# rkin100g/Nerf-Replication

Measured on AMD Instinct MI355X. Metric: rays/sec (800x800, 64+128 samples), higher is better.
Workload: dtype f32; 1 GPU; lego-shaped 800x800 frame = 640000 pinhole rays, 64 coarse + 128 fine hierarchical samples, 8+1-layer W=256 NeRF x2, seeded synthetic weights (latest.pth unavailable offline); BASELINE.json configs[1]; parallelism=ray-tile shard x1 (each rank generates and renders only its tile) + 1 all_gather

## Files before the change

nerf_replication_amd/csrc/nerf_frame.hip.inc:

```
#include "nerf_host.h"

namespace {

__global__ void nerf_occupancy_tally_kernel(const int* __restrict__ count, long long all, long long* __restrict__ evaluated) {
  *evaluated += count ? (long long)*count : all;
}

}

extern "C" {

static constexpr int64_t kRenderBlockRays = 1 << 20;
static int64_t render_block_rays() {
  const char* env = getenv("NERF_RENDER_BLOCK_RAYS");
  constexpr long long kMax = 0x7fffffff / (NERF_N_SAMPLES + NERF_N_IMPORTANCE);
  if (env) { const long long v = atoll(env); if (v >= 64) return (int64_t)(v < kMax ? v : kMax); }
  return kRenderBlockRays;
}

struct RenderWorkspace {
  float* raw_c; float* t_sorted = nullptr; float* raw_f = nullptr; uint8_t* valid = nullptr; int* index; int* count; float* t_jit = nullptr;
  uint8_t* valid_c = nullptr; int* index_c = nullptr;
  int64_t bytes;
  RenderWorkspace(void* base, int64_t n_rays, int32_t n_importance, int32_t fast_sampling, bool stochastic, bool occupancy = false) {
    Carver c(base);
    const int64_t S = NERF_N_SAMPLES + NERF_N_IMPORTANCE;
    raw_c = c.take<float>(n_rays * NERF_N_SAMPLES * 4);
    if (n_importance) {
      t_sorted = c.take<float>(n_rays * S);
      raw_f = c.take<float>(n_rays * S * 4);
    }
    if (n_importance && (fast_sampling || occupancy)) {
      valid = c.take<uint8_t>(n_rays * S);
      index = c.take<int>(n_rays * S);
    } else {
      index = c.take<int>(n_rays);
    }
    count = c.take<int>(1);
    if (stochastic) t_jit = c.take<float>(n_rays * NERF_N_SAMPLES);
    if (occupancy) {
      valid_c = c.take<uint8_t>(n_rays * NERF_N_SAMPLES);
      index_c = c.take<int>(n_rays * NERF_N_SAMPLES);
    }
    bytes = c.bytes();
  }
};
static int64_t render_workspace_bytes(int64_t n_rays_frame, int32_t n_importance, int32_t fast_sampling, bool stochastic,
                                      bool occupancy = false) {
  if (n_rays_frame < 0) return -1;
  const int64_t n_rays = n_rays_frame < render_block_rays() ? n_rays_frame : render_block_rays();
  return RenderWorkspace(nullptr, n_rays, n_importance, fast_sampling, stochastic, occupancy).bytes;
}

struct RenderOccupancy {
  const uint32_t* coarse; const uint32_t* fine;
  int32_t dims[3]; float box_min[3], inv_step[3];
  long long* evaluated;
};
static int occupancy_tally(const int* count, long long all, long long* evaluated, hipStream_t st) {
  return NERF_LAUNCH(nerf_occupancy_tally_kernel, dim3(1), dim3(1), st, count, all, evaluated);
}
int64_t nerf_render_workspace_bytes(int64_t n_rays_frame, int32_t n_importance, int32_t fast_sampling) {
  return render_workspace_bytes(n_rays_frame, n_importance, fast_sampling, false);
}
int64_t nerf_render_stochastic_workspace_bytes(int64_t n_rays_frame, int32_t n_importance) {
  return render_workspace_bytes(n_rays_frame, n_importance, 0, true);
}

static int32_t render_frame(const char* entry, const float* rays_o, const float* rays_d, int64_t n_rays, const void* packed_coarse,
                            const void* packed_fine, const float* t_coarse, const float* u, const float* jitter, const float* u_rays,
                            bool stochastic, int32_t n_importance, int32_t white_bkgd, int32_t precision, int32_t fast_sampling,
                            float weights_threshold, void* workspace, int64_t workspace_bytes, float* rgb, float* depth, void* stream,
                            const RenderOccupancy* occ = nullptr) {
  if (n_rays < 0) return fail(NERF_ERR_INVALID_ARG, "%s: bad size", entry);
  if (n_importance != 0 && n_importance != NERF_N_IMPORTANCE)
    return fail(NERF_ERR_INVALID_ARG, "%s: n_importance must be 0 or 128", entry);
  if (n_rays == 0) return NERF_OK;
  if (!rays_o || !rays_d || !packed_coarse || !t_coarse || !rgb || !depth || !workspace ||
      (n_importance && (!packed_fine || !u)))
    return fail(NERF_ERR_INVALID_ARG, "%s: null argument", entry);
  if (workspace_bytes < render_workspace_bytes(n_rays, n_importance, fast_sampling, stochastic, occ != nullptr))
    return fail(NERF_ERR_WORKSPACE, "%s: workspace too small", entry);
  const int64_t S = NERF_N_SAMPLES + NERF_N_IMPORTANCE;
  if (fast_sampling && n_importance && n_rays > (int64_t)0x7fffffff / S)
    return fail(NERF_ERR_INVALID_ARG, "%s: fast_sampling handles at most 11 184 810 rays per call "
                                      "(n_rays * 192 point ids must fit in int32): split the frame", entry);
  hipStream_t st = (hipStream_t)stream;
  const int64_t B = render_block_rays();
  for (int64_t r0 = 0; r0 < n_rays; r0 += B) {
    const int64_t nb = n_rays - r0 < B ? n_rays - r0 : B;
    const float* o = rays_o + 3 * r0;
    const float* d = rays_d + 3 * r0;
    float* rgb_b = rgb + 3 * r0;
    float* depth_b = depth + r0;
    const RenderWorkspace w(workspace, nb, n_importance, fast_sampling, stochastic, occ != nullptr);
    auto list_pass = [&](const uint8_t* valid, long long np, int* index, float* raw) -> int {
      if (hipMemsetAsync(w.count, 0, sizeof(int), st) != hipSuccess ||
          hipMemsetAsync(raw, 0, (size_t)(np * 4 * (int64_t)sizeof(float)), st) != hipSuccess)
        return fail(NERF_ERR_HIP, "%s: memset failed", entry);
      return NERF_LAUNCH(nerf_compact_kernel, dim3((unsigned)((np + 255) / 256)), dim3(256), st, valid, np, index, w.count);
    };
    auto tally = [&](int pass, bool listed, long long all) -> int {
      return occ && occ->evaluated ? occupancy_tally(listed ? w.count : nullptr, all, occ->evaluated + pass, st) : NERF_OK;
    };
    const float* tc = t_coarse;
    int64_t tcs = 0;
    int rc;
    if (jitter) {
      rc = nerf_stratified_samples(t_coarse, jitter + NERF_N_SAMPLES * r0, nb, w.t_jit, stream);
      if (rc) return rc;
      tc = w.t_jit; tcs = NERF_N_SAMPLES;
    }
    const bool cull_c = occ && occ->coarse;
    if (cull_c) {
      rc = nerf_occupancy_mark(o, d, tc, tcs, nb, NERF_N_SAMPLES, occ->coarse, occ->dims, occ->box_min, occ->inv_step, 0, w.valid_c, stream);
      if (rc) return rc;
      rc = list_pass(w.valid_c, nb * NERF_N_SAMPLES, w.index_c, w.raw_c);
      if (rc) return rc;
    }
    const bool fp16 = precision == NERF_PREC_F16 || precision == NERF_PREC_F16S;
    const bool exact_coarse = fp16 && fast_sampling && n_importance;
    rc = forward_rays(entry, o, d, tc, tcs, nb, NERF_N_SAMPLES, exact_coarse ? (const char*)packed_coarse + nerf::kF16PackedBytes : packed_coarse,
                      w.raw_c, false, nullptr, n_importance != 0, false, exact_coarse ? NERF_PREC_F32X : precision, stream,
                      cull_c ? w.index_c : nullptr, cull_c ? w.count : nullptr);
    if (rc) return rc;
    rc = tally(0, cull_c, nb * NERF_N_SAMPLES);
    if (rc) return rc;
    const bool guard = fp16 && nb <= (int64_t)0x7fffffff / S;
    auto far_plane_guard = [&](const float* tvals, int64_t stride, int32_t S_, const void* packed_f16, float* raw) -> int {
      if (const int r2 = NERF_LAUNCH(nerf_last_sample_index_kernel, dim3((unsigned)((nb + 255) / 256)), dim3(256), st, w.index, w.count,
                                     (long long)nb, S_)) return r2;
      return forward_rays(entry, o, d, tvals, stride, nb, S_, (const char*)packed_f16 + nerf::kF16PackedBytes, raw, false, nullptr, false,
                          false, NERF_PREC_F32X, stream, w.index, w.count);
    };
    if (n_importance == 0) {
      if (guard) {
        rc = far_plane_guard(tc, tcs, NERF_N_SAMPLES, packed_coarse, w.raw_c);
        if (rc) return rc;
      }
      rc = nerf_composite(w.raw_c, tc, tcs, nb, NERF_N_SAMPLES, white_bkgd, rgb_b, depth_b, nullptr, stream);
      if (rc) return rc;
      continue;
    }
    rc = nerf_sample_fine_rays(w.raw_c, tc, tcs, u_rays ? u_rays + NERF_N_IMPORTANCE * r0 : u, u_rays ? NERF_N_IMPORTANCE : 0, nb, w.t_sorted,
                               nullptr, fast_sampling ? w.valid : nullptr, fast_sampling ? weights_threshold : 0.f, fast_sampling ? 0.45f : 0.f,
                               stream);
    if (rc) return rc;
    const bool cull_f = occ && occ->fine;
    if (cull_f) {
      rc = nerf_occupancy_mark(o, d, w.t_sorted, S, nb, (int32_t)S, occ->fine, occ->dims, occ->box_min, occ->inv_step, fast_sampling != 0, w.valid,
                               stream);
      if (rc) return rc;
    }
    if (!fast_sampling && !cull_f) {
      rc = forward_rays(entry, o, d, w.t_sorted, S, nb, (int32_t)S, packed_fine, w.raw_f, false, nullptr, false, true, precision, stream);
      if (rc) return rc;
      if (guard) {
        rc = far_plane_guard(w.t_sorted, S, (int32_t)S, packed_fine, w.raw_f);
        if (rc) return rc;
      }
    } else {
      rc = list_pass(w.valid, nb * S, w.index, w.raw_f);
      if (rc) return rc;
      rc = forward_rays(entry, o, d, w.t_sorted, S, nb, (int32_t)S, packed_fine, w.raw_f, false, nullptr, false, true, precision, stream,
                        w.index, w.count);
      if (rc) return rc;
    }
    rc = tally(1, fast_sampling || cull_f, nb * S);
    if (rc) return rc;
    if (guard && fast_sampling && !cull_f) {
      rc = far_plane_guard(w.t_sorted, S, (int32_t)S, packed_fine, w.raw_f);
      if (rc) return rc;
    }
    rc = nerf_composite(w.raw_f, w.t_sorted, S, nb, (int32_t)S, white_bkgd, rgb_b, depth_b, nullptr, stream);
    if (rc) return rc;
  }
  return NERF_OK;
}

int32_t nerf_render_forward(const float* rays_o, const float* rays_d, int64_t n_rays,
                            const void* packed_coarse, const void* packed_fine,
                            const float* t_coarse, const float* u, int32_t n_importance,
                            int32_t white_bkgd, int32_t precision, int32_t fast_sampling,
                            float weights_threshold, void* workspace,
                            int64_t workspace_bytes, float* rgb, float* depth, void* stream) {
  return render_frame("nerf_render_forward", rays_o, rays_d, n_rays, packed_coarse, packed_fine, t_coarse, u, nullptr, nullptr, false,
                      n_importance, white_bkgd, precision, fast_sampling, weights_threshold, workspace, workspace_bytes, rgb, depth, stream);
}

int32_t nerf_render_forward_stochastic(const float* rays_o, const float* rays_d, int64_t n_rays,
                                       const void* packed_coarse, const void* packed_fine,
                                       const float* t_coarse, const float* u, const float* jitter, const float* u_rays,
                                       int32_t n_importance, int32_t white_bkgd, int32_t precision, int32_t fast_sampling,
                                       float weights_threshold, void* workspace, int64_t workspace_bytes,
                                       float* rgb, float* depth, void* stream) {
  if (precision != NERF_PREC_F32 && precision != NERF_PREC_F32X)
    return fail(NERF_ERR_INVALID_ARG, "%s", "nerf_render_forward_stochastic: precision must be f32 or f32x");
  if (fast_sampling) return fail(NERF_ERR_INVALID_ARG, "%s", "nerf_render_forward_stochastic: fast_sampling is not supported");
  return render_frame("nerf_render_forward_stochastic", rays_o, rays_d, n_rays, packed_coarse, packed_fine, t_coarse, u, jitter, u_rays,
                      true, n_importance, white_bkgd, precision, 0, weights_threshold, workspace, workspace_bytes, rgb, depth, stream);
}

}
```

nerf_replication_amd/csrc/nerf_mlp_common.h:

```cpp
#pragma once
#include <hip/hip_runtime.h>
#include <utility>

#include "nerf_layout.h"

typedef float f32x16 __attribute__((ext_vector_type(16)));
typedef float f32x4 __attribute__((ext_vector_type(4)));
typedef float f32x2 __attribute__((ext_vector_type(2)));
typedef unsigned u32x4 __attribute__((ext_vector_type(4)));
typedef _Float16 h8 __attribute__((ext_vector_type(8)));
typedef _Float16 h4 __attribute__((ext_vector_type(4)));
typedef _Float16 h2 __attribute__((ext_vector_type(2)));

typedef __attribute__((address_space(3))) void lds_void;
typedef const __attribute__((address_space(1))) void gbl_void;
typedef __attribute__((address_space(3))) char lds_char;
typedef __attribute__((address_space(3))) f32x4 lds_f32x4;
typedef const __attribute__((address_space(3))) float lds_cfloat;
typedef const __attribute__((address_space(3))) f32x2 lds_cf32x2;
typedef const __attribute__((address_space(3))) f32x4 lds_cf32x4;
typedef const __attribute__((address_space(3))) h8 lds_ch8;

constexpr int kF16Waves = 8;
constexpr int kF16Threads = kF16Waves * 64;
constexpr int kF16TilePts = kF16Waves * 32;
constexpr int kF16RingSlots = 4;
constexpr int kF16LdsBytes = nerf::kF16ConstBytes + kF16RingSlots * nerf::kF16ChunkBytes;
constexpr int kXWaves = 4;
constexpr int kXThreads = kXWaves * 64;
constexpr int kXTilePts = kXWaves * 32;

__device__ __forceinline__ f32x16 mfma32(float a, float b, f32x16 c) {
  return __builtin_amdgcn_mfma_f32_32x32x2f32(a, b, c, 0, 0, 0);
}
__device__ __forceinline__ f32x16 mfma16(h8 a, h8 b, f32x16 c) {
  return __builtin_amdgcn_mfma_f32_32x32x16_f16(a, b, c, 0, 0, 0);
}

__device__ __forceinline__ void sincos_cw(float x, float& s, float& c) {
  const float n = rintf(x * 0.636619772367581343f);
  float r = fmaf(n, -1.5703125f, x);
  r = fmaf(n, -4.837512969970703125e-4f, r);
  r = fmaf(n, -7.54978995489188216e-8f, r);
  const float r2 = r * r;
  const float sp = fmaf(r * r2, fmaf(r2, fmaf(r2, -1.9515295891e-4f, 8.3321608736e-3f), -1.6666654611e-1f), r);
  const float cp = fmaf(r2 * r2, fmaf(r2, fmaf(r2, 2.443315711809948e-5f, -1.388731625493765e-3f), 4.166664568298827e-2f),
                        fmaf(r2, -0.5f, 1.0f));
  const int q = (int)n;
  const float ss = (q & 1) ? cp : sp;
  const float cc = (q & 1) ? sp : cp;
  s = (q & 2) ? -ss : ss;
  c = ((q + 1) & 2) ? -cc : cc;
}

__device__ __forceinline__ int uniform_load_i32(const int* p) {
  return *(const __attribute__((address_space(4))) int*)p;
}

template <class F, int... I>
__device__ __forceinline__ void static_for_impl(F&& f, std::integer_sequence<int, I...>) { (f(std::integral_constant<int, I>{}), ...); }
template <int N, class F>
__device__ __forceinline__ void static_for(F&& f) { static_for_impl(f, std::make_integer_sequence<int, N>{}); }

struct MlpArgs {
  const float* pts;
  const float* rays_o;
  const float* rays_d;
  const float* viewdirs;
  const float* tvals;
  long long t_ray_stride;
  long long n_points;
  int n_samples;
  const float* packed;
  float* raw;
  const int* index;
  const int* count;
  float* save;
  int skip_dead_colour;
  int density_only;
  const float* fold;
  int skip_dead_ksteps;
  int skip_dead_groups;
};

struct TrainSave {
  static constexpr int kPe = 64, kDpe = 32;
  static constexpr long long pad32(long long P) { return (P + 31) & ~31LL; }
  static constexpr long long off_pe(long long P) { return 0; }
  static constexpr long long off_dpe(long long P) { return pad32(P) * 64; }
  static constexpr long long off_h(long long P, int l) { return pad32(P) * (96 + 256LL * l); }
  static constexpr long long off_f(long long P) { return pad32(P) * (96 + 2048); }
  static constexpr long long off_hv(long long P) { return pad32(P) * (96 + 2304); }
  static constexpr int kMasked = 9;
  static constexpr long long off_bits(long long P) { return pad32(P) * (96 + 2304 + 128); }
  static constexpr long long bits_block(long long tile, int which) { return ((tile * kMasked + which) * 64) * 4; }
  static constexpr long long off_stamp(long long P) { return off_bits(P) + (pad32(P) / 32) * kMasked * 256; }
  static constexpr long long floats(long long P) { return off_stamp(P) + 4; }
};

struct BwdArgs {
  const float* rays_o; const float* rays_d; const float* tvals; long long t_ray_stride;
  long long n_points; int n_samples;
  const float* packed_bwd;
  const float* draw;
  const float* save;
  float* gsave;
  float* g_t;
  const float* pts;
  float* g_x;
  int density_only;
  const int* live_tiles;
  const int* n_live;
};

struct TrainGrad {
  static constexpr long long off_gzv(long long P) { return 0; }
  static constexpr long long off_gf(long long P) { return TrainSave::pad32(P) * 128; }
  static constexpr long long off_gz(long long P, int l) { return TrainSave::pad32(P) * (384 + 256LL * (7 - l)); }
  static constexpr long long n_tiles(long long P) { return TrainSave::pad32(P) / 32; }
  static constexpr long long off_flags(long long P) { return TrainSave::pad32(P) * (384 + 2048); }
  static constexpr long long off_live(long long P) { return off_flags(P) + ((n_tiles(P) + 3) & ~3LL); }
  static constexpr long long off_count(long long P) { return off_live(P) + ((n_tiles(P) + 3) & ~3LL); }
  static constexpr long long floats(long long P) { return off_count(P) + 4; }
};
```

nerf_replication_amd/csrc/nerf_mlp_f32.hip.inc:

```

#include "nerf_mlp_common.h"

#ifndef NERF_F32_WG_WAVES
#define NERF_F32_WG_WAVES 1
#endif
#ifndef NERF_F32_HACK_NOBIAS
#define NERF_F32_HACK_NOBIAS 0
#endif
#ifndef NERF_F32_HACK_NOSAVE
#define NERF_F32_HACK_NOSAVE 0
#endif
#ifndef NERF_BWD_HACK_NOMASK
#define NERF_BWD_HACK_NOMASK 0
#endif

constexpr int kTailFloats = 3072;
static_assert(nerf::kOffHeadBias - nerf::kOffBias == kTailFloats, "LDS tail = biases + views bias + head weights");
template <int NT>
__device__ __forceinline__ void load_bias(f32x16 (&acc)[NT], lds_cfloat* bias_h) {
  lds_cf32x4* b = reinterpret_cast<lds_cf32x4*>(bias_h);
#pragma unroll
  for (int j = 0; j < NT; ++j) {
#pragma unroll
    for (int q = 0; q < 4; ++q) {
      f32x4 v = NERF_F32_HACK_NOBIAS ? f32x4{0.f, 0.f, 0.f, 0.f} : b[j * 4 + q];
      acc[j][4 * q + 0] = v.x; acc[j][4 * q + 1] = v.y; acc[j][4 * q + 2] = v.z; acc[j][4 * q + 3] = v.w;
    }
  }
}

constexpr int kRing = 16;
constexpr int kPF = 8;

#ifndef NERF_SAVE_TAPS
#define NERF_SAVE_TAPS 1
#endif
struct NoTap { static constexpr bool kIsTap = false; __device__ __forceinline__ void operator()(int, int, const f32x16&) const {} };
struct SignBits { unsigned w0 = 0u, w1 = 0u, w2 = 0u, w3 = 0u; };
template <bool GRAD, bool BITS = false>
struct StoreTap {
  static constexpr bool kIsTap = true;
  float* row;
  SignBits* sb;
  __device__ __forceinline__ void operator()(int t, int q, const f32x16& Xt) const {
    f32x4 v;
    v.x = Xt[4 * q + 0]; v.y = Xt[4 * q + 1]; v.z = Xt[4 * q + 2]; v.w = Xt[4 * q + 3];
    asm volatile("" : "+v"(v));
    if (!(GRAD ? 0 : NERF_F32_HACK_NOSAVE)) {
      *reinterpret_cast<f32x4*>(row + 32 * t + 8 * q) = v;
    }
    if constexpr (BITS) {
      auto nz = [](float x) { const unsigned u = __float_as_uint(x); return u < 1u ? u : 1u; };
      const unsigned m = (nz(v.x) | (nz(v.y) << 1) | (nz(v.z) << 2) | (nz(v.w) << 3)) << (16 * (t & 1) + 4 * q);
      switch (t >> 1) {
        case 0: sb->w0 |= m; break;
        case 1: sb->w1 |= m; break;
        case 2: sb->w2 |= m; break;
        default: sb->w3 |= m; break;
      }
    }
  }
};
template <bool ON, bool BITS>
__device__ __forceinline__ auto save_tap(float* row, SignBits* sb) {
  if constexpr (ON && NERF_SAVE_TAPS) return StoreTap<false, BITS>{row, sb};
  else return NoTap{};
}

struct AStream {
  const char* base;
  unsigned voff;
  f32x4 ring[kRing];
};
template <int N, int K = 0>
__device__ __forceinline__ void astream_load(AStream& as, int first, int slot0) {
  if constexpr (K < N) {
    const char* b = as.base + (long long)(first + (K & ~3)) * 1024;
    asm volatile("global_load_dwordx4 %0, %1, %2 offset:%3"
                 : "=&v"(as.ring[(slot0 + K) % kRing]) : "v"(as.voff), "s"(b), "n"((K & 3) * 1024) : "memory");
    astream_load<N, K + 1>(as, first, slot0);
  }
}
template <int K>
__device__ __forceinline__ void astream_load_one(AStream& as, int first, int slot0) {
  const char* b = as.base + (long long)(first + (K & ~3)) * 1024;
  asm volatile("global_load_dwordx4 %0, %1, %2 offset:%3"
               : "=&v"(as.ring[(slot0 + K) % kRing]) : "v"(as.voff), "s"(b), "n"((K & 3) * 1024) : "memory");
}
__device__ __forceinline__ void astream_fetch_from(AStream& as, unsigned& P) {
  const char* b0 = as.base + (long long)P * (8 * 1024);
  const char* b1 = b0 + 4096;
  asm volatile("s_cmp_eq_u32 %[P], 0\n\t"
               "s_cbranch_scc1 .Lpre_done_%=\n\t"
               "s_waitcnt vmcnt(0)\n\t"
               "s_bitcmp1_b32 %[P], 0\n\t"
               "s_cbranch_scc1 .Lpre_odd_%=\n\t"
               "global_load_dwordx4 %0, %[vo], %[b0]\n\t"
               "global_load_dwordx4 %1, %[vo], %[b0] offset:1024\n\t"
               "global_load_dwordx4 %2, %[vo], %[b0] offset:2048\n\t"
               "global_load_dwordx4 %3, %[vo], %[b0] offset:3072\n\t"
               "global_load_dwordx4 %4, %[vo], %[b1]\n\t"
               "global_load_dwordx4 %5, %[vo], %[b1] offset:1024\n\t"
               "global_load_dwordx4 %6, %[vo], %[b1] offset:2048\n\t"
               "global_load_dwordx4 %7, %[vo], %[b1] offset:3072\n\t"
               "s_branch .Lpre_done_%=\n"
               ".Lpre_odd_%=:\n\t"
               "global_load_dwordx4 %8, %[vo], %[b0]\n\t"
               "global_load_dwordx4 %9, %[vo], %[b0] offset:1024\n\t"
               "global_load_dwordx4 %10, %[vo], %[b0] offset:2048\n\t"
               "global_load_dwordx4 %11, %[vo], %[b0] offset:3072\n\t"
               "global_load_dwordx4 %12, %[vo], %[b1]\n\t"
               "global_load_dwordx4 %13, %[vo], %[b1] offset:1024\n\t"
               "global_load_dwordx4 %14, %[vo], %[b1] offset:2048\n\t"
               "global_load_dwordx4 %15, %[vo], %[b1] offset:3072\n"
               ".Lpre_done_%=:"
               : "+v"(as.ring[0]), "+v"(as.ring[1]), "+v"(as.ring[2]), "+v"(as.ring[3]), "+v"(as.ring[4]), "+v"(as.ring[5]),
                 "+v"(as.ring[6]), "+v"(as.ring[7]), "+v"(as.ring[8]), "+v"(as.ring[9]), "+v"(as.ring[10]), "+v"(as.ring[11]),
                 "+v"(as.ring[12]), "+v"(as.ring[13]), "+v"(as.ring[14]), "+v"(as.ring[15]), [P] "+s"(P)
               : [vo] "v"(as.voff), [b0] "s"(b0), [b1] "s"(b1) : "memory", "scc");
}
template <int N, int CNT = 8>
__device__ __forceinline__ void astream_wait(AStream& as, int slot0) {
  static_assert(N == 2 || N == 4 || N == 8, "blocks per k-group");
  static_assert(CNT >= 0 && CNT <= 9, "outstanding operations allowed");
  if constexpr (N == 8)
    asm volatile("s_waitcnt vmcnt(%8)"
                 : "+v"(as.ring[(slot0 + 0) % kRing]), "+v"(as.ring[(slot0 + 1) % kRing]), "+v"(as.ring[(slot0 + 2) % kRing]),
                   "+v"(as.ring[(slot0 + 3) % kRing]), "+v"(as.ring[(slot0 + 4) % kRing]), "+v"(as.ring[(slot0 + 5) % kRing]),
                   "+v"(as.ring[(slot0 + 6) % kRing]), "+v"(as.ring[(slot0 + 7) % kRing]) : "n"(CNT) : "memory");
  else if constexpr (N == 4)
    asm volatile("s_waitcnt vmcnt(%4)"
                 : "+v"(as.ring[(slot0 + 0) % kRing]), "+v"(as.ring[(slot0 + 1) % kRing]), "+v"(as.ring[(slot0 + 2) % kRing]),
                   "+v"(as.ring[(slot0 + 3) % kRing]) : "n"(CNT) : "memory");
  else
    asm volatile("s_waitcnt vmcnt(%2)" : "+v"(as.ring[(slot0 + 0) % kRing]), "+v"(as.ring[(slot0 + 1) % kRing]) : "n"(CNT) : "memory");
}
__device__ __forceinline__ void stream_drain(AStream& as) {
  asm volatile("s_waitcnt vmcnt(0)"
               : "+v"(as.ring[0]), "+v"(as.ring[1]), "+v"(as.ring[2]), "+v"(as.ring[3]), "+v"(as.ring[4]), "+v"(as.ring[5]),
                 "+v"(as.ring[6]), "+v"(as.ring[7]), "+v"(as.ring[8]), "+v"(as.ring[9]), "+v"(as.ring[10]), "+v"(as.ring[11]),
                 "+v"(as.ring[12]), "+v"(as.ring[13]), "+v"(as.ring[14]), "+v"(as.ring[15]) :: "memory");
}
__device__ __forceinline__ void stream_reassert_uniform(AStream& as) {
  const unsigned long long b = reinterpret_cast<unsigned long long>(as.base);
  const unsigned lo = __builtin_amdgcn_readfirstlane((unsigned)b), hi = __builtin_amdgcn_readfirstlane((unsigned)(b >> 32));
  as.base = reinterpret_cast<const char*>(((unsigned long long)hi << 32) | lo);
}
__device__ __forceinline__ void wstream_start(AStream& as, const f32x4* p_lane0, int lane) {
  as.base = reinterpret_cast<const char*>(p_lane0);
  as.voff = (unsigned)lane * 16u;
  astream_load<8>(as, 0, 0);
}
__device__ __forceinline__ unsigned long long kstep_live(float x, unsigned kthr) {
  return __builtin_amdgcn_ballot_w64(__float_as_uint(x) >= kthr);
}
#ifndef NERF_F32_ASM_OVERRUN
#define NERF_F32_ASM_OVERRUN 0
#endif
__device__ __forceinline__ bool group_dead(const unsigned long long (&live4)[4]) {
  return ((live4[0] | live4[1]) | (live4[2] | live4[3])) == 0ull;
}
template <int KT, int NT, bool LAST = false, class TAP = NoTap, bool KSKIP = false>
__device__ __forceinline__ void gemm_tiles(f32x16 (&acc)[NT], const f32x16 (&X)[KT], AStream& as, TAP tap = TAP(), unsigned kthr = 0u,
                                           bool prefix = false) {
  static_assert(kRing == 16 && kPF == 8, "interleaved form: ring 16, 8 blocks in flight");
  static_assert(!KSKIP || !TAP::kIsTap, "k-step skipping: inference instances only");
  static_assert((KT * 4 * NT) % kRing == 0, "layer steps must be a multiple of the ring");
  static_assert(!LAST || (kPF % NT == 0 && KT * 4 * NT >= 2 * kPF), "tail handling: whole groups");
  constexpr int kBlocks = KT * 4 * NT;
  constexpr bool kPrefix = KSKIP && NT == 8 && !(LAST && NERF_F32_ASM_OVERRUN);
  unsigned P = 0u;
  if constexpr (kPrefix) {
#pragma unroll
    for (int k = kRing / 2; k < kRing; ++k) asm volatile("" : "=v"(as.ring[k]));
    if (prefix) {
#pragma unroll
      for (int g = 0; g + 1 < KT * 4; ++g) {
        unsigned long long live4[4];
#pragma unroll
        for (int q = 0; q < 4; ++q) live4[q] = kstep_live(X[g >> 2][(g & 3) * 4 + q], kthr);
        if (!group_dead(live4)) break;
        P = g + 1;
      }
    }
    astream_fetch_from(as, P);
  }
  if constexpr (KSKIP) {
    if constexpr (NT == 8)
      asm volatile("" : "+a"(acc[0]), "+a"(acc[1]), "+a"(acc[2]), "+a"(acc[3]), "+a"(acc[4 % NT]), "+a"(acc[5 % NT]), "+a"(acc[6 % NT]), "+a"(acc[7 % NT]));
    else
      asm volatile("" : "+a"(acc[0]), "+a"(acc[1]), "+a"(acc[2]), "+a"(acc[3]));
  }
#pragma unroll
  for (int g = 0; g < KT * 4; ++g) {
    if constexpr (NT == 8 && !TAP::kIsTap && !(LAST && NERF_F32_ASM_OVERRUN)) {
      const bool kMore = !LAST || g * NT + kPF < kBlocks;
      const int t = g >> 2, r0 = (g & 3) * 4;
      if constexpr (KSKIP) {
        if (g + 1 < KT * 4 && (unsigned)g < P) continue;
      }
      astream_wait<NT, 0>(as, (g * NT) % kRing);
      __builtin_amdgcn_sched_barrier(0);
      tap(t, g & 3, X[t]);
      unsigned long long live4[4] = {0ull, 0ull, 0ull, 0ull};
      if constexpr (KSKIP) {
#pragma unroll
        for (int q = 0; q < 4; ++q) live4[q] = kstep_live(X[t][r0 + q], kthr);
        __builtin_amdgcn_sched_barrier(0);
      }
#pragma unroll
      for (int q = 0; q < 4; ++q) {
        if constexpr (KSKIP) {
          unsigned long long live = live4[q];
          if (q == 0 && kMore) {
#pragma unroll
            for (int j = 0; j < 4; ++j) {
              asm volatile("" : "+s"(live));
              if (live) acc[j] = mfma32(as.ring[(g * NT + j) % kRing][0], X[t][r0], acc[j]);
              __builtin_amdgcn_sched_barrier(0);
              if (j == 0) { astream_load_one<0>(as, g * NT + kPF, (g * NT + kPF) % kRing); astream_load_one<1>(as, g * NT + kPF, (g * NT + kPF) % kRing); }
              if (j == 1) { astream_load_one<2>(as, g * NT + kPF, (g * NT + kPF) % kRing); astream_load_one<3>(as, g * NT + kPF, (g * NT + kPF) % kRing); }
              if (j == 2) { astream_load_one<4>(as, g * NT + kPF, (g * NT + kPF) % kRing); astream_load_one<5>(as, g * NT + kPF, (g * NT + kPF) % kRing); }
              if (j == 3) { astream_load_one<6>(as, g * NT + kPF, (g * NT + kPF) % kRing); astream_load_one<7>(as, g * NT + kPF, (g * NT + kPF) % kRing); }
              __builtin_amdgcn_sched_barrier(0);
            }
            asm volatile("" : "+s"(live));
            if (live) {
#pragma unroll
              for (int j = 4; j < NT; ++j) acc[j] = mfma32(as.ring[(g * NT + j) % kRing][0], X[t][r0], acc[j]);
            }
          } else if (live) {
#pragma unroll
            for (int j = 0; j < NT; ++j) acc[j] = mfma32(as.ring[(g * NT + j) % kRing][q], X[t][r0 + q], acc[j]);
          }
          continue;
        }
#pragma unroll
        for (int j = 0; j < NT; ++j) {
          const f32x4 a = as.ring[(g * NT + j) % kRing];
          acc[j] = mfma32(a[q], X[t][r0 + q], acc[j]);
          if (q == 0 && j < 4 && kMore) {
            __builtin_amdgcn_sched_barrier(0);
            if (j == 0) { astream_load_one<0>(as, g * NT + kPF, (g * NT + kPF) % kRing); astream_load_one<1>(as, g * NT + kPF, (g * NT + kPF) % kRing); }
            if (j == 1) { astream_load_one<2>(as, g * NT + kPF, (g * NT + kPF) % kRing); astream_load_one<3>(as, g * NT + kPF, (g * NT + kPF) % kRing); }
            if (j == 2) { astream_load_one<4>(as, g * NT + kPF, (g * NT + kPF) % kRing); astream_load_one<5>(as, g * NT + kPF, (g * NT + kPF) % kRing); }
            if (j == 3) { astream_load_one<6>(as, g * NT + kPF, (g * NT + kPF) % kRing); astream_load_one<7>(as, g * NT + kPF, (g * NT + kPF) % kRing); }
            __builtin_amdgcn_sched_barrier(0);
          }
        }
      }
      __builtin_amdgcn_sched_barrier(0);
      continue;
    } else if constexpr (!LAST || NERF_F32_ASM_OVERRUN) {
      astream_load<NT>(as, g * NT + kPF, (g * NT + kPF) % kRing);
      if (g == 0) astream_wait<NT>(as, (g * NT) % kRing);
      else astream_wait<NT, kPF>(as, (g * NT) % kRing);
    } else {
      if (g * NT + kPF < kBlocks) astream_load<NT>(as, g * NT + kPF, (g * NT + kPF) % kRing);
      const int younger = kBlocks - (g + 1) * NT < kPF ? kBlocks - (g + 1) * NT : kPF;
      switch (younger) {
        case 8: astream_wait<NT, 8>(as, (g * NT) % kRing); break;
        case 6: astream_wait<NT, 6>(as, (g * NT) % kRing); break;
        case 4: astream_wait<NT, 4>(as, (g * NT) % kRing); break;
        case 2: astream_wait<NT, 2>(as, (g * NT) % kRing); break;
        default: astream_wait<NT, 0>(as, (g * NT) % kRing); break;
      }
    }
    __builtin_amdgcn_sched_barrier(0);
    const int t = g >> 2, r0 = (g & 3) * 4;
    tap(t, g & 3, X[t]);
#pragma unroll
    for (int q = 0; q < 4; ++q) {
      if constexpr (KSKIP) {
        if (!kstep_live(X[t][r0 + q], kthr)) continue;
      }
#pragma unroll
      for (int j = 0; j < NT; ++j) {
        const f32x4 a = as.ring[(g * NT + j) % kRing];
        acc[j] = mfma32(a[q], X[t][r0 + q], acc[j]);
      }
    }
    __builtin_amdgcn_sched_barrier(0);
  }
  as.base += (long long)KT * 4 * NT * 1024;
}

template <int NT>
__device__ __forceinline__ u32x4 relu_bits_tiles(f32x16 (&acc)[NT]) {
  unsigned w[4] = {0u, 0u, 0u, 0u};
#pragma unroll
  for (int j = 0; j < NT; ++j)
#pragma unroll
    for (int r = 0; r < 16; ++r) {
      const int v = __float_as_int(acc[j][r]);
      const int rl = v > 0 ? v : 0;
      acc[j][r] = __int_as_float(rl);
      w[j >> 1] |= ((unsigned)rl < 1u ? 0u : 1u) << (16 * (j & 1) + r);
    }
  u32x4 b; b.x = w[0]; b.y = w[1]; b.z = w[2]; b.w = w[3];
  return b;
}
template <int NT>
__device__ __forceinline__ void relu_tiles(f32x16 (&acc)[NT]) {
#pragma unroll
  for (int j = 0; j < NT; ++j)
#pragma unroll
    for (int r = 0; r < 16; ++r) {
      const int bits = __float_as_int(acc[j][r]);
      acc[j][r] = __int_as_float(bits > 0 ? bits : 0);
    }
}

template <bool RAY_MODE, bool SAVE = false, bool DENS = false, bool DSKIP = false>
__global__ __launch_bounds__(256) __attribute__((amdgpu_waves_per_eu(1, 1)))
void nerf_mlp_f32_kernel(MlpArgs a) {
  static_assert(!(DSKIP && DENS), "dead-colour skipping is a variant of the full network");
  using namespace nerf;
  const int lane = threadIdx.x & 63;
  const int wave = threadIdx.x >> 6;
  const int h = lane >> 5;
  const long long n_points = a.index ? (long long)*a.count : a.n_points;
  const long long base = ((long long)blockIdx.x * (blockDim.x >> 6) + wave) * kTilePts;
  if (base >= n_points) return;
  {
  const long long pl = base + (lane & 31);
  const bool valid = pl < n_points;
  const long long plc = valid ? pl : n_points - 1;
  const long long p = a.index ? (long long)a.index[plc] : plc;
  const long long pc = p;
  const long long ray = pc / a.n_samples;
  const int s = (int)(pc - ray * a.n_samples);

  constexpr int kTailLds = kTailFloats + (DENS ? 0 : 256);
  __shared__ __attribute__((aligned(16))) float tail_smem[NERF_F32_WG_WAVES * kTailLds];
  lds_char* const tail_w = (lds_char*)tail_smem + wave * (kTailLds * 4);
  {
    const char* src = reinterpret_cast<const char*>(a.packed + kOffBias) + lane * 16;
#pragma unroll
    for (int i = 0; i < kTailFloats * 4 / 1024; ++i)
      __builtin_amdgcn_global_load_lds((gbl_void*)(src + i * 1024),
                                       (lds_void*)(tail_w + i * 1024), 16, 0, 0);
    if constexpr (!DENS)
      __builtin_amdgcn_global_load_lds((gbl_void*)(reinterpret_cast<const char*>(a.fold + kFoldOffBias) + lane * 16),
                                       (lds_void*)(tail_w + kTailFloats * 4), 16, 0, 0);
  }
  lds_cfloat* const tail = reinterpret_cast<lds_cfloat*>(tail_w);

  float x[3], d[3];
  if (RAY_MODE) {
    const float t = a.tvals[ray * a.t_ray_stride + s];
#pragma unroll
    for (int c = 0; c < 3; ++c) {
      const float dc = a.rays_d[ray * 3 + c];
      x[c] = __fadd_rn(a.rays_o[ray * 3 + c], __fmul_rn(dc, t));
      d[c] = dc;
    }
  } else {
#pragma unroll
    for (int c = 0; c < 3; ++c) x[c] = a.pts[pc * 3 + c];
  }
  if (a.viewdirs != nullptr) {
#pragma unroll
    for (int c = 0; c < 3; ++c) d[c] = a.viewdirs[ray * 3 + c];
  } else {
    const float n2 = __fadd_rn(__fadd_rn(__fmul_rn(d[0], d[0]), __fmul_rn(d[1], d[1])), __fmul_rn(d[2], d[2]));
    const float nrm = __fsqrt_rn(n2);
#pragma unroll
    for (int c = 0; c < 3; ++c) d[c] = __fdiv_rn(d[c], nrm);
  }

  f32x16 PE[2], DPE[1];
  {
    const float hs = h ? 32.0f : 1.0f;
#pragma unroll
    for (int ai = 0; ai < 15; ++ai) {
      const float arg = x[ai % 3] * (hs * (float)(1 << (ai / 3)));
      float sv, cv;
      sincosf(arg, &sv, &cv);
      PE[(2 * ai) >> 4][(2 * ai) & 15] = sv;
      PE[(2 * ai + 1) >> 4][(2 * ai + 1) & 15] = cv;
    }
    PE[1][14] = h ? x[2] : x[0];
    PE[1][15] = h ? 0.0f : x[1];
  }
  auto encode_dir = [&]() {
    const float ds = h ? 4.0f : 1.0f;
#pragma unroll
    for (int ai = 0; ai < 6; ++ai) {
      const float arg = d[ai % 3] * (ds * (float)(1 << (ai / 3)));
      float sv, cv;
      sincosf(arg, &sv, &cv);
      DPE[0][2 * ai] = sv;
      DPE[0][2 * ai + 1] = cv;
    }
    DPE[0][12] = h ? d[2] : d[0];
    DPE[0][13] = h ? 0.0f : d[1];
    DPE[0][14] = 0.0f;
    DPE[0][15] = 0.0f;
  };
  const long long ps = pl;
  if (SAVE) encode_dir();
  if (SAVE && !NERF_F32_HACK_NOSAVE) {
    float* pe_row = a.save + TrainSave::off_pe(a.n_points) + ps * 64;
#pragma unroll
    for (int n = 0; n < 32; ++n) {
      const int c0 = pe_xyz_feat(n, 0), c1 = pe_xyz_feat(n, 1);
      const int c = h ? c1 : c0;
      if (c >= 0) pe_row[c] = PE[n >> 4][n & 15];
    }
    if (h) pe_row[63] = 0.0f;
    float* dpe_row = a.save + TrainSave::off_dpe(a.n_points) + ps * 32;
#pragma unroll
    for (int n = 0; n < 16; ++n) {
      const int c0 = pe_dir_feat(n, 0), c1 = pe_dir_feat(n, 1);
      const int c = h ? c1 : c0;
      if (c >= 0) dpe_row[c] = DPE[0][n];
    }
    if (h) { dpe_row[27] = 0.f; dpe_row[28] = 0.f; dpe_row[29] = 0.f; dpe_row[30] = 0.f; dpe_row[31] = 0.f; }
  }

  const float* __restrict__ pk = a.packed;
  AStream ws;
  asm volatile("s_waitcnt vmcnt(0)" ::: "memory");
  wstream_start(ws, reinterpret_cast<const f32x4*>(pk), lane);
  lds_cfloat* bias = tail + h * 128;

  float* const srow = SAVE ? a.save + ps * 256 + 4 * h : nullptr;
  u32x4* const bits_out = SAVE ? reinterpret_cast<u32x4*>(a.save + TrainSave::off_bits(a.n_points) +
                                                          TrainSave::bits_block(base / kTilePts, 0)) + lane : nullptr;
  SignBits sb;
  constexpr bool kTapBits = SAVE;
  auto tap_bits_done = [&](int which) {
    if constexpr (kTapBits) {
      u32x4 b; b.x = sb.w0; b.y = sb.w1; b.z = sb.w2; b.w = sb.w3;
      if (!NERF_F32_HACK_NOSAVE) bits_out[which * 64] = b;
      sb = SignBits();
    }
  };
  auto relu8 = [&](f32x16 (&A)[8], int which) {
    relu_tiles<8>(A);
  };

  constexpr bool kKSkip = !SAVE;
  const unsigned kthr = a.skip_dead_ksteps ? 1u : 0u;
  const bool kpre = a.skip_dead_ksteps && a.skip_dead_groups;
  using TrunkTap = decltype(save_tap<SAVE, kTapBits>(srow, &sb));

  f32x16 X[8], Y[8];
  load_bias<8>(X, bias);
  gemm_tiles<2, 8>(X, PE, ws);
  relu8(X, 0);

  float sigma = 0.0f;
  constexpr int kPairs = 3;
#pragma unroll 1
  for (int pr = 0; pr < kPairs; ++pr) {
    load_bias<8>(Y, bias + (1 + 2 * pr) * 256);
    if (pr == 2) {
      gemm_tiles<2, 8>(Y, PE, ws);
    }
    gemm_tiles<8, 8, false, TrunkTap, kKSkip>(Y, X, ws, save_tap<SAVE, kTapBits>(srow + TrainSave::off_h(a.n_points, 2 * pr), &sb), kthr, kpre);
    tap_bits_done(2 * pr);
    relu8(Y, 1 + 2 * pr);
    load_bias<8>(X, bias + (2 + 2 * pr) * 256);
    gemm_tiles<8, 8, false, TrunkTap, kKSkip>(X, Y, ws, save_tap<SAVE, kTapBits>(srow + TrainSave::off_h(a.n_points, 1 + 2 * pr), &sb), kthr, kpre);
    tap_bits_done(1 + 2 * pr);
    relu8(X, 2 + 2 * pr);
  }

  if constexpr (DENS) {
    load_bias<8>(Y, bias + 7 * 256);
    gemm_tiles<8, 8, true, TrunkTap, kKSkip>(Y, X, ws, save_tap<SAVE, kTapBits>(srow + TrainSave::off_h(a.n_points, 6), &sb), kthr, kpre);
    tap_bits_done(6);
    relu8(Y, 7);
    lds_cf32x4* wa = reinterpret_cast<lds_cf32x4*>(tail + (kOffWAlpha - kOffBias) + h * 128);
    float acc0 = 0.f, acc1 = 0.f, acc2 = 0.f, acc3 = 0.f;
#pragma unroll
    for (int t = 0; t < 8; ++t)
#pragma unroll
      for (int q = 0; q < 4; ++q) {
        const f32x4 w4 = wa[t * 4 + q];
        acc0 = fmaf(w4.x, Y[t][4 * q + 0], acc0);
        acc1 = fmaf(w4.y, Y[t][4 * q + 1], acc1);
        acc2 = fmaf(w4.z, Y[t][4 * q + 2], acc2);
        acc3 = fmaf(w4.w, Y[t][4 * q + 3], acc3);
      }
    sigma = (acc0 + acc1) + (acc2 + acc3);
    if constexpr (SAVE) {
      StoreTap<false, kTapBits> tap{srow + TrainSave::off_h(a.n_points, 7), &sb};
#pragma unroll
      for (int t = 0; t < 8; ++t)
#pragma unroll
        for (int q = 0; q < 4; ++q) tap(t, q, Y[t]);
      tap_bits_done(7);
    }
    f32x4 out;
    out.x = 0.0f; out.y = 0.0f; out.z = 0.0f;
    out.w = sigma + __shfl_xor(sigma, 32) + pk[kOffHeadBias + 3];
    if (valid && h == 0) reinterpret_cast<f32x4*>(a.raw)[p] = out;
    return;
  }

  load_bias<8>(Y, bias + 7 * 256);
  gemm_tiles<8, 8, !SAVE, TrunkTap, kKSkip>(Y, X, ws, save_tap<SAVE, kTapBits>(srow + TrainSave::off_h(a.n_points, 6), &sb), kthr, kpre);
  tap_bits_done(6);
  relu8(Y, 7);
  stream_drain(ws);
  {
    lds_cf32x4* wa = reinterpret_cast<lds_cf32x4*>(tail + (kOffWAlpha - kOffBias) + h * 128);
    float acc0 = 0.f, acc1 = 0.f, acc2 = 0.f, acc3 = 0.f;
#pragma unroll
    for (int t = 0; t < 8; ++t)
#pragma unroll
      for (int q = 0; q < 4; ++q) {
        const f32x4 w4 = wa[t * 4 + q];
        acc0 = fmaf(w4.x, Y[t][4 * q + 0], acc0);
        acc1 = fmaf(w4.y, Y[t][4 * q + 1], acc1);
        acc2 = fmaf(w4.z, Y[t][4 * q + 2], acc2);
        acc3 = fmaf(w4.w, Y[t][4 * q + 3], acc3);
      }
    sigma = (acc0 + acc1) + (acc2 + acc3);
  }
  bool live_tile = true;
  if constexpr (DSKIP) {
    const float sigma_full = sigma + __shfl_xor(sigma, 32) + pk[kOffHeadBias + 3];
    live_tile = __builtin_amdgcn_readfirstlane((int)(__builtin_amdgcn_ballot_w64(valid && sigma_full > 0.0f) != 0ull)) != 0;
  }

  float rgb[3] = {0.0f, 0.0f, 0.0f};
  if (!DSKIP || live_tile) {
  if constexpr (SAVE) {
    load_bias<8>(X, bias + 8 * 256);
    gemm_tiles<8, 8, true>(X, Y, ws, save_tap<SAVE, kTapBits>(srow + TrainSave::off_h(a.n_points, 7), &sb));
    tap_bits_done(7);
    StoreTap<false> ftap{srow + TrainSave::off_f(a.n_points), nullptr};
#pragma unroll
    for (int t = 0; t < 8; ++t)
#pragma unroll
      for (int q = 0; q < 4; ++q) ftap(t, q, X[t]);
  }
  f32x16 V[4];
  if (!SAVE) encode_dir();
  wstream_start(ws, reinterpret_cast<const f32x4*>(a.fold + kFoldOffWvf), lane);
  load_bias<4>(V, tail + kTailFloats + h * 64);
  gemm_tiles<8, 4, false, NoTap, kKSkip>(V, Y, ws, NoTap(), kthr);
  gemm_tiles<1, 4, true>(V, DPE, ws);
  if constexpr (SAVE) {
    const u32x4 b = relu_bits_tiles<4>(V);
    if (!NERF_F32_HACK_NOSAVE) bits_out[8 * 64] = b;
    StoreTap<false> tap{a.save + TrainSave::off_hv(a.n_points) + ps * 128 + 4 * h, nullptr};
#pragma unroll
    for (int t = 0; t < 4; ++t)
#pragma unroll
      for (int q = 0; q < 4; ++q) tap(t, q, V[t]);
  } else relu_tiles<4>(V);

#pragma unroll
  for (int c = 0; c < 3; ++c) {
    lds_cf32x4* wr = reinterpret_cast<lds_cf32x4*>(tail + (kOffWRgb - kOffBias) + (c * 2 + h) * 64);
    float acc0 = 0.f, acc1 = 0.f, acc2 = 0.f, acc3 = 0.f;
#pragma unroll
    for (int t = 0; t < 4; ++t)
#pragma unroll
      for (int q = 0; q < 4; ++q) {
        const f32x4 w4 = wr[t * 4 + q];
        acc0 = fmaf(w4.x, V[t][4 * q + 0], acc0);
        acc1 = fmaf(w4.y, V[t][4 * q + 1], acc1);
        acc2 = fmaf(w4.z, V[t][4 * q + 2], acc2);
        acc3 = fmaf(w4.w, V[t][4 * q + 3], acc3);
      }
    rgb[c] = (acc0 + acc1) + (acc2 + acc3);
  }
#pragma unroll
  for (int c = 0; c < 3; ++c) rgb[c] = rgb[c] + __shfl_xor(rgb[c], 32) + pk[kOffHeadBias + c];
  }
  f32x4 out;
  out.x = rgb[0];
  out.y = rgb[1];
  out.z = rgb[2];
  out.w = sigma + __shfl_xor(sigma, 32) + pk[kOffHeadBias + 3];
  if (valid && h == 0) reinterpret_cast<f32x4*>(a.raw)[p] = out;
  }
}
```

nerf_replication_amd/csrc/nerf_mlp_launch.hip.inc:

```
#include "nerf_host.h"
#include "nerf_mlp_common.h"

namespace {

bool dead_tile_list_available(long long P, int precision) {
  const char* env = getenv("NERF_DEAD_TILE_SKIP");
  const bool want = !(env && env[0] == '0');
  return want && (precision == NERF_PREC_F32 || precision == NERF_PREC_F32X) && P % 32 == 0 && P / 32 <= 0x7fffffffLL;
}

int dead_kstep_skip_wanted() {
  const char* env = getenv("NERF_DEAD_KSTEP_SKIP");
  return !(env && env[0] == '0');
}

int dead_group_skip_wanted() {
  const char* env = getenv("NERF_DEAD_GROUP_SKIP");
  return dead_kstep_skip_wanted() && !(env && env[0] == '0');
}

}

extern "C" {

using MlpKernel = void (*)(MlpArgs);
struct MlpFamily {
  const char* name;
  int wg_pts, threads;
  bool persistent;
  MlpKernel inst[4];
};
#define NERF_MLP_INFERENCE_3(K) {K<true, true>, K<true, false, true>, K<true>, K<false>}
#define NERF_MLP_INFERENCE_4(K) {K<true, false, true>, K<true, false, false, true>, K<true>, K<false>}
#define NERF_MLP_SAVE(K) {K<true, true, true>, K<true, true, false, true>, K<true, true>, K<false, true>}
static const MlpFamily kMlpF32x = {"nerf_mlp_f32x_kernel", kXTilePts, kXThreads, true, NERF_MLP_INFERENCE_4(nerf_mlp_f32x_kernel)};
static const MlpFamily kMlpF16s = {"nerf_mlp_f16s_kernel", kF16TilePts, kF16Threads, true, NERF_MLP_INFERENCE_3(nerf_mlp_f16s_kernel)};
static const MlpFamily kMlpF16 = {"nerf_mlp_f16_kernel", kF16TilePts, kF16Threads, true, NERF_MLP_INFERENCE_3(nerf_mlp_f16_kernel)};
static const MlpFamily kMlpF32 = {"nerf_mlp_f32_kernel", nerf::kTilePts * NERF_F32_WG_WAVES, 64 * NERF_F32_WG_WAVES, false,
                           NERF_MLP_INFERENCE_4(nerf_mlp_f32_kernel)};
static const MlpFamily kMlpSaveF32x = {"nerf_mlp_f32x_kernel", kXTilePts, kXThreads, true, NERF_MLP_SAVE(nerf_mlp_f32x_kernel)};
static const MlpFamily kMlpSaveF32 = {"nerf_mlp_f32_kernel", nerf::kTilePts, 64, false, NERF_MLP_SAVE(nerf_mlp_f32_kernel)};
static const MlpFamily* mlp_family(int precision, bool save) {
  switch (precision) {
    case NERF_PREC_F32: return save ? &kMlpSaveF32 : &kMlpF32;
    case NERF_PREC_F32X: return save ? &kMlpSaveF32x : &kMlpF32x;
    case NERF_PREC_F16: return save ? nullptr : &kMlpF16;
    case NERF_PREC_F16S: return save ? nullptr : &kMlpF16s;
  }
  return nullptr;
}

static unsigned persistent_blocks(long long n_points, int wg_pts) {
  const long long n_tiles = (n_points + wg_pts - 1) / wg_pts;
  return (unsigned)(n_tiles < num_cus() ? n_tiles : num_cus());
}

static int launch_mlp(const MlpArgs& a_in, bool ray_mode, bool save, int precision, hipStream_t st, const char* entry) {
  if (!mlp_family(precision, false)) return fail(NERF_ERR_UNSUPPORTED, "%s: precision not built", entry);
  if (a_in.n_points <= 0) return NERF_OK;
  MlpArgs a = a_in;
  if (a.index && a.n_points > 0x7fffffffLL) return fail(NERF_ERR_INVALID_ARG, "%s: index mode: point ids are int32", entry);
  const MlpFamily* f = mlp_family(precision, save);
  if (!f) return fail(NERF_ERR_UNSUPPORTED, "%s: f32 or f32x only", entry);
  const MlpKernel k = f->inst[!ray_mode ? 3 : a.density_only ? 0 : a.skip_dead_colour ? 1 : 2];
  if (precision == NERF_PREC_F32) a.fold = a.packed + nerf::kOffFold;
  a.skip_dead_ksteps = dead_kstep_skip_wanted();
  a.skip_dead_groups = dead_group_skip_wanted();
  if (f->persistent) return launch(f->name, k, dim3(persistent_blocks(a.n_points, f->wg_pts)), dim3(f->threads), st, a);
  const long long blocks = (a.n_points + f->wg_pts - 1) / f->wg_pts;
  if (blocks > 0x7fffffffLL) return fail(NERF_ERR_INVALID_ARG, "%s: too many points for one launch", entry);
  return launch(f->name, k, dim3((unsigned)blocks), dim3(f->threads), st, a);
}

static int forward_rays(const char* entry, const float* rays_o, const float* rays_d, const float* tvals, int64_t t_ray_stride, int64_t n_rays,
                        int32_t n_samples, const void* packed, float* raw, bool want_save, float* save, bool density_only,
                        bool for_compositing, int32_t precision, void* stream, const int* index = nullptr, const int* count = nullptr) {
  if (n_rays < 0 || n_samples <= 0 || t_ray_stride < 0) return fail(NERF_ERR_INVALID_ARG, "%s: bad size", entry);
  if (n_rays == 0) return NERF_OK;
  if (!rays_o || !rays_d || !tvals || !packed || !raw || (want_save && !save)) return fail(NERF_ERR_INVALID_ARG, "%s: null argument", entry);
  MlpArgs a{};
  a.rays_o = rays_o; a.rays_d = rays_d; a.tvals = tvals; a.t_ray_stride = t_ray_stride;
  a.n_points = n_rays * n_samples; a.n_samples = n_samples; a.packed = (const float*)packed; a.raw = raw; a.save = save;
  a.density_only = density_only; a.skip_dead_colour = for_compositing;
  a.index = index; a.count = count;
  if (want_save) {
    a.skip_dead_colour = for_compositing && dead_tile_list_available(a.n_points, precision);
    if (hipMemsetAsync(save + TrainSave::off_stamp(a.n_points), a.skip_dead_colour ? 0x01 : 0x00, 4 * sizeof(float), (hipStream_t)stream) != hipSuccess)
      return fail(NERF_ERR_HIP, "%s: memset failed", entry);
  }
  return launch_mlp(a, true, want_save, precision, (hipStream_t)stream, entry);
}

int32_t nerf_mlp_forward(const float* pts, const float* viewdirs, int64_t n_rays, int32_t n_samples,
                         const void* packed, float* raw, int32_t precision, void* stream) {
  if (n_rays < 0 || n_samples <= 0) return fail(NERF_ERR_INVALID_ARG, "%s", "nerf_mlp_forward: bad size");
  if (n_rays == 0) return NERF_OK;
  if (!pts || !viewdirs || !packed || !raw) return fail(NERF_ERR_INVALID_ARG, "%s", "nerf_mlp_forward: null argument");
  MlpArgs a{};
  a.pts = pts; a.viewdirs = viewdirs; a.n_points = n_rays * n_samples; a.n_samples = n_samples;
  a.packed = (const float*)packed; a.raw = raw;
  return launch_mlp(a, false, false, precision, (hipStream_t)stream, "nerf_mlp_forward");
}

int32_t nerf_mlp_forward_rays(const float* rays_o, const float* rays_d, const float* tvals,
                              int64_t t_ray_stride, int64_t n_rays, int32_t n_samples,
                              const void* packed, float* raw, int32_t precision, void* stream) {
  return forward_rays("nerf_mlp_forward_rays", rays_o, rays_d, tvals, t_ray_stride, n_rays, n_samples, packed, raw, false, nullptr,
                      false, false, precision, stream);
}

int32_t nerf_mlp_forward_rays_for_compositing(const float* rays_o, const float* rays_d, const float* tvals,
                                              int64_t t_ray_stride, int64_t n_rays, int32_t n_samples,
                                              const void* packed, float* raw, int32_t precision, void* stream) {
  return forward_rays("nerf_mlp_forward_rays_for_compositing", rays_o, rays_d, tvals, t_ray_stride, n_rays, n_samples, packed, raw,
                      false, nullptr, false, true, precision, stream);
}

int32_t nerf_mlp_forward_rays_density(const float* rays_o, const float* rays_d, const float* tvals,
                                      int64_t t_ray_stride, int64_t n_rays, int32_t n_samples,
                                      const void* packed, float* raw, int32_t precision, void* stream) {
  return forward_rays("nerf_mlp_forward_rays_density", rays_o, rays_d, tvals, t_ray_stride, n_rays, n_samples, packed, raw, false,
                      nullptr, true, false, precision, stream);
}

int64_t nerf_train_save_floats(int64_t n_points) { return n_points < 0 ? -1 : TrainSave::floats(n_points); }

int32_t nerf_mlp_forward_rays_save(const float* rays_o, const float* rays_d, const float* tvals,
                                   int64_t t_ray_stride, int64_t n_rays, int32_t n_samples,
                                   const void* packed, float* raw, float* save, int32_t precision, void* stream) {
  return forward_rays("nerf_mlp_forward_rays_save", rays_o, rays_d, tvals, t_ray_stride, n_rays, n_samples, packed, raw, true, save,
                      false, false, precision, stream);
}
int32_t nerf_mlp_forward_rays_save_for_compositing(const float* rays_o, const float* rays_d, const float* tvals,
                                                   int64_t t_ray_stride, int64_t n_rays, int32_t n_samples,
                                                   const void* packed, float* raw, float* save, int32_t precision, void* stream) {
  return forward_rays("nerf_mlp_forward_rays_save_for_compositing", rays_o, rays_d, tvals, t_ray_stride, n_rays, n_samples, packed,
                      raw, true, save, false, true, precision, stream);
}
int32_t nerf_mlp_forward_rays_save_density(const float* rays_o, const float* rays_d, const float* tvals,
                                           int64_t t_ray_stride, int64_t n_rays, int32_t n_samples,
                                           const void* packed, float* raw, float* save, int32_t precision, void* stream) {
  return forward_rays("nerf_mlp_forward_rays_save_density", rays_o, rays_d, tvals, t_ray_stride, n_rays, n_samples, packed, raw, true,
                      save, true, false, precision, stream);
}

static bool masked_sizes_ok(int64_t n_rays, int32_t n_samples, int64_t t_ray_stride) {
  return n_rays >= 0 && n_samples > 0 && t_ray_stride >= 0 && n_rays <= (int64_t)0x7fffffff / n_samples;
}

int32_t nerf_mlp_forward_rays_save_masked(const float* rays_o, const float* rays_d, const float* tvals, int64_t t_ray_stride,
                                          int64_t n_rays, int32_t n_samples, const int32_t* index, const int32_t* count,
                                          const void* packed, float* raw, float* save, int32_t precision, void* stream) {
  if (!masked_sizes_ok(n_rays, n_samples, t_ray_stride)) return fail(NERF_ERR_INVALID_ARG, "%s", "nerf_mlp_forward_rays_save_masked: bad size");
  if (n_rays == 0) return NERF_OK;
  if (!index || !count) return fail(NERF_ERR_INVALID_ARG, "%s", "nerf_mlp_forward_rays_save_masked: null argument");
  return forward_rays("nerf_mlp_forward_rays_save_masked", rays_o, rays_d, tvals, t_ray_stride, n_rays, n_samples, packed, raw, true,
                      save, false, true, precision, stream, index, count);
}

int32_t nerf_mlp_forward_points_save(const float* pts, const float* viewdirs, int64_t n_rays, int32_t n_samples,
                                     const void* packed, float* raw, float* save, int32_t precision, void* stream) {
  if (n_rays < 0 || n_samples <= 0) return fail(NERF_ERR_INVALID_ARG, "%s", "nerf_mlp_forward_points_save: bad size");
  if (n_rays == 0) return NERF_OK;
  if (!pts || !viewdirs || !packed || !raw || !save) return fail(NERF_ERR_INVALID_ARG, "%s", "nerf_mlp_forward_points_save: null argument");
  MlpArgs a{};
  a.pts = pts; a.viewdirs = viewdirs; a.n_points = n_rays * n_samples; a.n_samples = n_samples;
  a.packed = (const float*)packed; a.raw = raw; a.save = save;
  if (hipMemsetAsync(save + TrainSave::off_stamp(a.n_points), 0, 4 * sizeof(float), (hipStream_t)stream) != hipSuccess)
    return fail(NERF_ERR_HIP, "%s", "nerf_mlp_forward_points_save: memset failed");
  return launch_mlp(a, false, true, precision, (hipStream_t)stream, "nerf_mlp_forward_points_save");
}

}
```

Before: 741,800 rays/s.

## Tile f32 MLP points as 8 rays by 4 samples per wave in render

Adds a tile_rays_log2 mode to the f32 ray-mode MLP kernel. Each 32-point wave tile now covers several rays with a few consecutive samples each, instead of 32 consecutive samples of one ray. The render path enables this by default with 8 rays per tile, and an env var can override it. The apparent aim is more coherent positions within a tile, so dead-group and dead-kstep skipping fires more often, and better locality. The cost is extra index arithmetic, a padded grid, and strided writes across rays.

```diff
diff --git a/nerf_replication_amd/csrc/nerf_frame.hip.inc b/nerf_replication_amd/csrc/nerf_frame.hip.inc
--- a/nerf_replication_amd/csrc/nerf_frame.hip.inc
+++ b/nerf_replication_amd/csrc/nerf_frame.hip.inc
@@ -122,7 +122,7 @@
     const bool exact_coarse = fp16 && fast_sampling && n_importance;
     rc = forward_rays(entry, o, d, tc, tcs, nb, NERF_N_SAMPLES, exact_coarse ? (const char*)packed_coarse + nerf::kF16PackedBytes : packed_coarse,
                       w.raw_c, false, nullptr, n_importance != 0, false, exact_coarse ? NERF_PREC_F32X : precision, stream,
-                      cull_c ? w.index_c : nullptr, cull_c ? w.count : nullptr);
+                      cull_c ? w.index_c : nullptr, cull_c ? w.count : nullptr, kRenderTileRaysLog2);
     if (rc) return rc;
     rc = tally(0, cull_c, nb * NERF_N_SAMPLES);
     if (rc) return rc;
@@ -153,7 +153,8 @@
       if (rc) return rc;
     }
     if (!fast_sampling && !cull_f) {
-      rc = forward_rays(entry, o, d, w.t_sorted, S, nb, (int32_t)S, packed_fine, w.raw_f, false, nullptr, false, true, precision, stream);
+      rc = forward_rays(entry, o, d, w.t_sorted, S, nb, (int32_t)S, packed_fine, w.raw_f, false, nullptr, false, true, precision, stream, nullptr,
+                        nullptr, kRenderTileRaysLog2);
       if (rc) return rc;
       if (guard) {
         rc = far_plane_guard(w.t_sorted, S, (int32_t)S, packed_fine, w.raw_f);
diff --git a/nerf_replication_amd/csrc/nerf_mlp_common.h b/nerf_replication_amd/csrc/nerf_mlp_common.h
--- a/nerf_replication_amd/csrc/nerf_mlp_common.h
+++ b/nerf_replication_amd/csrc/nerf_mlp_common.h
@@ -71,6 +71,7 @@
   long long t_ray_stride;
   long long n_points;
   int n_samples;
+  int tile_rays_log2;
   const float* packed;
   float* raw;
   const int* index;
diff --git a/nerf_replication_amd/csrc/nerf_mlp_f32.hip.inc b/nerf_replication_amd/csrc/nerf_mlp_f32.hip.inc
--- a/nerf_replication_amd/csrc/nerf_mlp_f32.hip.inc
+++ b/nerf_replication_amd/csrc/nerf_mlp_f32.hip.inc
@@ -320,16 +320,34 @@
   const int wave = threadIdx.x >> 6;
   const int h = lane >> 5;
   const long long n_points = a.index ? (long long)*a.count : a.n_points;
-  const long long base = ((long long)blockIdx.x * (blockDim.x >> 6) + wave) * kTilePts;
-  if (base >= n_points) return;
+  const long long tile = (long long)blockIdx.x * (blockDim.x >> 6) + wave;
+  const long long base = tile * kTilePts;
+  const int lg = (RAY_MODE && !SAVE) ? a.tile_rays_log2 : 0;
+  const long long pl = base + (lane & 31);
+  long long p, ray;
+  int s;
+  bool valid;
+  if (lg != 0) {
+    const long long n_rays = n_points / a.n_samples;
+    const int q = a.n_samples >> (5 - lg);
+    const long long g = tile / q;
+    if ((g << lg) >= n_rays) return;
+    const int j = lane & 31;
+    const long long r = (g << lg) + (j >> (5 - lg));
+    valid = r < n_rays;
+    ray = valid ? r : n_rays - 1;
+    s = ((int)(tile - g * q) << (5 - lg)) + (j & ((32 >> lg) - 1));
+    p = ray * a.n_samples + s;
+  } else {
+    if (base >= n_points) return;
+    valid = pl < n_points;
+    const long long plc = valid ? pl : n_points - 1;
+    p = a.index ? (long long)a.index[plc] : plc;
+    ray = p / a.n_samples;
+    s = (int)(p - ray * a.n_samples);
+  }
   {
-  const long long pl = base + (lane & 31);
-  const bool valid = pl < n_points;
-  const long long plc = valid ? pl : n_points - 1;
-  const long long p = a.index ? (long long)a.index[plc] : plc;
   const long long pc = p;
-  const long long ray = pc / a.n_samples;
-  const int s = (int)(pc - ray * a.n_samples);
 
   constexpr int kTailLds = kTailFloats + (DENS ? 0 : 256);
   __shared__ __attribute__((aligned(16))) float tail_smem[NERF_F32_WG_WAVES * kTailLds];
diff --git a/nerf_replication_amd/csrc/nerf_mlp_launch.hip.inc b/nerf_replication_amd/csrc/nerf_mlp_launch.hip.inc
--- a/nerf_replication_amd/csrc/nerf_mlp_launch.hip.inc
+++ b/nerf_replication_amd/csrc/nerf_mlp_launch.hip.inc
@@ -17,6 +17,18 @@
 int dead_group_skip_wanted() {
   const char* env = getenv("NERF_DEAD_GROUP_SKIP");
   return dead_kstep_skip_wanted() && !(env && env[0] == '0');
+}
+
+constexpr int kRenderTileRaysLog2 = 3;
+int tile_rays_log2_wanted(int dflt) {
+  const char* env = getenv("NERF_TILE_RAYS");
+  if (!env) return dflt;
+  for (int lg = 0; lg <= 5; ++lg) {
+    char want[4];
+    snprintf(want, sizeof want, "%d", 1 << lg);
+    if (!strcmp(env, want)) return lg;
+  }
+  return dflt;
 }
 
 }
@@ -67,14 +79,20 @@
   a.skip_dead_ksteps = dead_kstep_skip_wanted();
   a.skip_dead_groups = dead_group_skip_wanted();
   if (f->persistent) return launch(f->name, k, dim3(persistent_blocks(a.n_points, f->wg_pts)), dim3(f->threads), st, a);
-  const long long blocks = (a.n_points + f->wg_pts - 1) / f->wg_pts;
+  long long grid_pts = a.n_points;
+  if (a.tile_rays_log2) {
+    const long long R = 1LL << a.tile_rays_log2;
+    grid_pts = (a.n_points / a.n_samples + R - 1) / R * R * a.n_samples;
+  }
+  const long long blocks = (grid_pts + f->wg_pts - 1) / f->wg_pts;
   if (blocks > 0x7fffffffLL) return fail(NERF_ERR_INVALID_ARG, "%s: too many points for one launch", entry);
   return launch(f->name, k, dim3((unsigned)blocks), dim3(f->threads), st, a);
 }
 
 static int forward_rays(const char* entry, const float* rays_o, const float* rays_d, const float* tvals, int64_t t_ray_stride, int64_t n_rays,
                         int32_t n_samples, const void* packed, float* raw, bool want_save, float* save, bool density_only,
-                        bool for_compositing, int32_t precision, void* stream, const int* index = nullptr, const int* count = nullptr) {
+                        bool for_compositing, int32_t precision, void* stream, const int* index = nullptr, const int* count = nullptr,
+                        int tile_rays_log2 = 0) {
   if (n_rays < 0 || n_samples <= 0 || t_ray_stride < 0) return fail(NERF_ERR_INVALID_ARG, "%s: bad size", entry);
   if (n_rays == 0) return NERF_OK;
   if (!rays_o || !rays_d || !tvals || !packed || !raw || (want_save && !save)) return fail(NERF_ERR_INVALID_ARG, "%s: null argument", entry);
@@ -83,6 +101,8 @@
   a.n_points = n_rays * n_samples; a.n_samples = n_samples; a.packed = (const float*)packed; a.raw = raw; a.save = save;
   a.density_only = density_only; a.skip_dead_colour = for_compositing;
   a.index = index; a.count = count;
+  const int lg = tile_rays_log2_wanted(tile_rays_log2);
+  a.tile_rays_log2 = precision == NERF_PREC_F32 && !index && !want_save && n_samples % (32 >> lg) == 0 ? lg : 0;
   if (want_save) {
     a.skip_dead_colour = for_compositing && dead_tile_list_available(a.n_points, precision);
     if (hipMemsetAsync(save + TrainSave::off_stamp(a.n_points), a.skip_dead_colour ? 0x01 : 0x00, 4 * sizeof(float), (hipStream_t)stream) != hipSuccess)
```

Measured after the change: 785,300 rays/s (median of 6 runs). 5.9% higher.
